# gardnerzhou/CHAP

Measured on AMD Instinct MI355X. Metric: training volumes/sec (2D 256^2 bs24), higher is better.
Workload: dtype bf16; 1 GPU; ACDC 2D DualDecoder bs=24 (12 lab + 12 unlab) 256x256, 1 perturb step(s), N_v=U; global_batch=24, parallelism=dp1, hip_graph=True, losses_finite=True

## Files before the change

### chap_amd/_lib.py

```python
import ctypes as C
import os

_HERE = os.path.dirname(os.path.abspath(__file__))
LIB_PATH = os.environ.get("CHAP_LIBPATH") or os.path.join(_HERE, "libchap_hip.so")

F32, BF16 = 0, 1
STATS_MAX_SLOTS, STATS_HDR = 1024, 4
ACT_BWD_SLOTS = 1024
LOSS_SLOTS, CHANSUM_SLOTS, L2NORM_SLOTS = 512, 512, 256
PACK_CONV_FWD, PACK_CONV_DGRAD, PACK_DECONV_FWD, PACK_DECONV_DGRAD, PACK_DOWN_DGRAD = range(5)

_vp, _i32, _i64, _f32, _sz = C.c_void_p, C.c_int32, C.c_int64, C.c_float, C.c_size_t


class Src(C.Structure):
    _fields_ = [("ptr", _vp), ("scale", _vp), ("shift", _vp), ("keep", _vp), ("chan_mul", _vp),
                ("C", _i32), ("ld", _i32), ("coff", _i32), ("act", _i32), ("slope", _f32), ("keep_scale", _f32)]


class ConvParams(C.Structure):
    _fields_ = [("src", Src * 2), ("nsrc", _i32), ("combine", _i32),
                ("N", _i32), ("D", _i32), ("H", _i32), ("W", _i32), ("ID", _i32), ("IH", _i32), ("IW", _i32),
                ("ksize", _i32), ("stride", _i32), ("dims", _i32),
                ("wpacked", _vp), ("bias", _vp), ("out", _vp),
# ... 70 lines not shown

class ChanSumParams(C.Structure):
    _fields_ = [("r", Src), ("out", _vp), ("npix", _i64), ("pix_per_sample", _i64), ("dtype", _i32), ("ws", _vp)]


class ClToPlanarParams(C.Structure):
    _fields_ = [("r", Src), ("out", _vp), ("N", _i32), ("P", _i32), ("dtype", _i32)]


class MixLossParams(C.Structure):
    _fields_ = [("logits", _vp), ("target_a", _vp), ("target_b", _vp), ("mask", _vp), ("w_a", _f32), ("w_b", _f32),
                ("acc", _vp), ("loss", _vp), ("dlogits", _vp), ("gscale", _f32), ("accumulate", _i32),
                ("N", _i32), ("C", _i32), ("P", _i32), ("smooth", _f32), ("k_dice", _f32), ("k_ce", _f32), ("gscale_dev", _vp)]


class PseudoParams(C.Structure):
    _fields_ = [("logits1", _vp), ("logits2", _vp), ("soft1", _vp), ("soft2", _vp), ("arg1", _vp), ("arg2", _vp),
                ("knowledge", _vp), ("N", _i32), ("C", _i32), ("P", _i32)]


class KlParams(C.Structure):
    _fields_ = [("logits", _vp * 2), ("target", _vp * 2), ("loss", _vp), ("dlogits", _vp * 2),
                ("gscale", _f32), ("gscale_dev", _vp), ("N", _i32), ("C", _i32), ("P", _i32), ("mode", _i32), ("ws", _vp)]


class EnsembleParams(C.Structure):
    _fields_ = [("logits1", _vp), ("logits2", _vp), ("prob", _vp), ("label", _vp), ("N", _i32), ("C", _i32), ("P", C.c_int64), ("mode", _i32)]


class WindowAccParams(C.Structure):
# ... 34 lines not shown
                ("probs_out", _vp), ("inv_npix", _f32), ("nchunk", _i32), ("B", _i32), ("U", _i32), ("C", _i32),
                ("mode", _i32), ("comp", _i32), ("branch", _i32), ("prob_kind", _i32)]


class FoldParams(C.Structure):
    _fields_ = [("g", _vp), ("mul", _vp), ("out", _vp), ("B", _i32), ("U", _i32), ("C", _i32), ("ld", _i32), ("coff", _i32),
                ("pix_per_sample", _i64), ("dtype", _i32)]


class BoxMixParams(C.Structure):
    _fields_ = [("a", _vp), ("b", _vp), ("out", _vp), ("box", _vp), ("N", _i32), ("H", _i32), ("W", _i32), ("is_i64", _i32), ("D", _i32)]


class BoxMaskParams(C.Structure):
    _fields_ = [("mask", _vp), ("box", _vp), ("N", _i32), ("H", _i32), ("W", _i32), ("D", _i32)]


class LccParams(C.Structure):
    _fields_ = [("labels", _vp), ("out", _vp), ("ws", _vp), ("N", _i32), ("H", _i32), ("W", _i32), ("num_classes", _i32), ("D", _i32)]


class DiffMaskParams(C.Structure):
    _fields_ = [("p1", _vp), ("p2", _vp), ("knowledge", _vp), ("out", _vp), ("pooled_ws", _vp),
                ("N", _i32), ("H", _i32), ("W", _i32), ("scale", _i32), ("k", _i32)]


class MetricResult(C.Structure):
    _fields_ = [("n_a", _i64), ("n_b", _i64), ("n_ab", _i64), ("n_ab_s", _i64), ("n_ba_s", _i64), ("q_lo", _i64), ("q_hi", _i64),
                ("sum_ab", C.c_double), ("sum_ba", C.c_double), ("max2_ab", C.c_double), ("max2_ba", C.c_double),
                ("v2_lo", C.c_double), ("v2_hi", C.c_double)]
# ... 41 lines not shown
_SIGS = {
    "chap_conv_fwd": ConvParams, "chap_pack_weights": PackParams, "chap_conv_c1_fwd": ConvC1Params,
    "chap_conv_c1_bwd": ConvC1BwdParams, "chap_wgrad": WgradParams, "chap_bn_finalize": BnFinalizeParams,
    "chap_bn_eval_affine": BnEvalParams, "chap_act_bwd_reduce": ActBwdParams, "chap_act_bwd_apply": ActBwdParams,
    "chap_act_pool2": PoolParams, "chap_upsample2x": UpsampleParams, "chap_upsample2x_bwd": UpsampleBwdParams,
    "chap_planar_to_cl": PlanarToClParams, "chap_channel_sum": ChanSumParams, "chap_cl_to_planar": ClToPlanarParams,
    "chap_ensemble_argmax": EnsembleParams, "chap_window_accumulate": WindowAccParams, "chap_window_finalize": WindowFinParams,
    "chap_mix_loss_fwd": MixLossParams, "chap_mix_loss_bwd": MixLossParams, "chap_pseudo_block": PseudoParams,
    "chap_kl_fwd_bwd": KlParams, "chap_l2_normalize": L2NormParams, "chap_perturb": AxpyParams,
    "chap_rand_uniform": RandParams, "chap_keep_mask": KeepMaskParams, "chap_chan_mask": ChanMaskParams,
    "chap_box_mix": BoxMixParams, "chap_box_mask": BoxMaskParams, "chap_largest_cc": LccParams,
    "chap_diff_mask": DiffMaskParams, "chap_sgd_step": SgdParams,
    "chap_sample_channel_sum": SampleChanSumParams, "chap_channel_drop": ChannelDropParams,
    "chap_fold_perturbed": FoldParams, "chap_grad_sim": GradSimParams, "chap_metrics": MetricsParams,
    "chap_augment2d": Augment2dParams, "chap_augment3d": Augment3dParams,
}
_SIZE_FNS = {"chap_pack_size": PackParams, "chap_conv_c1_bwd_ws": ConvC1BwdParams, "chap_wgrad_ws": WgradParams,
             "chap_lcc_ws": LccParams, "chap_metrics_ws": MetricsParams}

_lib = None


ABI_VERSION = 9


class ChapError(RuntimeError):
    pass


def lib():
# ... 134 lines not shown
```

### chap_amd/csrc/aux.hip

```cpp
#include "common.h"
#include "launch.h"

__global__ __launch_bounds__(256) void l2norm_sumsq_kernel(const float* __restrict__ in, float* __restrict__ ss, int P) {
    __shared__ float red[4];
    const float* x = in + (long)blockIdx.y * P;
    float s = 0.f;
    for (int i = blockIdx.x * 256 + threadIdx.x; i < P; i += gridDim.x * 256) { const float v = x[i]; s += v * v; }
    s = wave_sum(s);
    if ((threadIdx.x & 63) == 0) red[threadIdx.x >> 6] = s;
    __syncthreads();
    if (threadIdx.x == 0) ss[(long)blockIdx.y * CHAP_L2NORM_SLOTS + blockIdx.x] = (red[0] + red[1]) + (red[2] + red[3]);
}
__global__ __launch_bounds__(256) void l2norm_scale_kernel(const float* __restrict__ in, float* __restrict__ out, const float* __restrict__ ss, int P, float eps) {
    __shared__ float tot;
    if (threadIdx.x < 64) {
        double t = 0.0;
        for (int b = threadIdx.x; b < (int)gridDim.x; b += 64) t += (double)ss[(long)blockIdx.y * CHAP_L2NORM_SLOTS + b];
#pragma unroll
        for (int o = 32; o > 0; o >>= 1) t += __shfl_xor(t, o, 64);
        if (threadIdx.x == 0) tot = (float)t;
    }
    __syncthreads();
    const float inv = 1.f / (sqrtf(tot) + eps);
    const float* x = in + (long)blockIdx.y * P;
// ... 101 lines not shown
__global__ void boxmask_kernel(const chap_boxmask_params P, int D) {
    const long total = (long)P.N * D * P.H * P.W;
    for (long i = (long)blockIdx.x * blockDim.x + threadIdx.x; i < total; i += (long)gridDim.x * blockDim.x) {
        const unsigned ui = (unsigned)i;
        const int x = (int)(ui % (unsigned)P.W), y = (int)((ui / (unsigned)P.W) % (unsigned)P.H), z = (int)((ui / (unsigned)(P.W * P.H)) % (unsigned)D);
        P.mask[i] = in_box(P.box, D, z, y, x) ? 0 : 1;
    }
}
extern "C" int chap_box_mask(const chap_boxmask_params* p, void* stream) {
    CHAP_CHECK_ARG(p && p->mask && p->box, "chap_box_mask: null argument");
    const int D = p->D > 1 ? p->D : 1;
    const long total = (long)p->N * D * p->H * p->W;
    const int nb = chap_blocks(total, 2048);
    hipLaunchKernelGGL(boxmask_kernel, dim3(nb), dim3(256), 0, (hipStream_t)stream, *p, D);
    CHAP_LAUNCH_CHECK("chap_box_mask");
    return CHAP_OK;
}

__global__ void diffmask_pool_kernel(const chap_diffmask_params P) {
    const int PH = P.H / P.scale, PW = P.W / P.scale;
    const long total = (long)P.N * PH * PW;
    for (long i = (long)blockIdx.x * blockDim.x + threadIdx.x; i < total; i += (long)gridDim.x * blockDim.x) {
        const int px = (int)(i % PW), py = (int)((i / PW) % PH), n = (int)(i / ((long)PW * PH));
        float s = 0.f;
        for (int dy = 0; dy < P.scale; ++dy)
            for (int dx = 0; dx < P.scale; ++dx) s += P.knowledge[((long)n * P.H + py * P.scale + dy) * P.W + px * P.scale + dx];
        P.pooled_ws[i] = s / (float)(P.scale * P.scale);
    }
}
__global__ __launch_bounds__(1024) void diffmask_select_kernel(const chap_diffmask_params P, float* thr_out) {
// ... 149 lines not shown
```

### chap_amd/csrc/loss.hip

```cpp
#include "common.h"

__device__ __forceinline__ double wave_sum_f64(double v) {
#pragma unroll
    for (int o = 32; o > 0; o >>= 1) v += __shfl_xor(v, o, 64);
    return v;
}
__device__ __forceinline__ void sum_partial_rows(float* ws, int nrows, int rl, float* tot) {
    const int wave = threadIdx.x >> 6, lane = threadIdx.x & 63;
    if (rl <= 32 && nrows <= CHAP_LOSS_SLOTS) {
        constexpr int NR = 8, NB = CHAP_LOSS_SLOTS / 64;
        float v[NR][NB];
#pragma unroll
        for (int r = 0; r < NR; ++r) {
            const int i = wave + 4 * r;
#pragma unroll
            for (int k = 0; k < NB; ++k) {
                const int b = lane + 64 * k;
                v[r][k] = ws[(long)(1 + (b < nrows ? b : 0)) * rl + (i < rl ? i : 0)];
            }
        }
#pragma unroll
        for (int r = 0; r < NR; ++r) {
            const int i = wave + 4 * r;
            double t = 0.0;
// ... 18 lines not shown
template <int C>
__device__ __forceinline__ void softmax_px(const float* __restrict__ lg, long base, long P, float z[C], float p[C], float& lse) {
    float m = -INFINITY;
#pragma unroll
    for (int c = 0; c < C; ++c) { z[c] = lg[base + c * P]; m = fmaxf(m, z[c]); }
    float s = 0.f;
#pragma unroll
    for (int c = 0; c < C; ++c) { p[c] = expf(z[c] - m); s += p[c]; }
    const float inv = 1.f / s;
#pragma unroll
    for (int c = 0; c < C; ++c) p[c] *= inv;
    lse = m + logf(s);
}

template <int C>
__global__ __launch_bounds__(256) void mix_loss_acc_kernel(const chap_mix_loss_params P_) {
    constexpr int NA = 2 + 3 * C;
    __shared__ float red[4][2 * NA];
    float a[2][NA];
#pragma unroll
    for (int k = 0; k < 2; ++k)
#pragma unroll
        for (int i = 0; i < NA; ++i) a[k][i] = 0.f;
    const long P = P_.P, total = (long)P_.N * P;
    for (long i = (long)blockIdx.x * 256 + threadIdx.x; i < total; i += (long)gridDim.x * 256) {
        const long n = (unsigned)i / (unsigned)P, pp = (unsigned)i % (unsigned)P;
        float z[C], p[C], lse;
        softmax_px<C>(P_.logits, n * C * P + pp, P, z, p, lse);
        const float m = P_.mask ? (float)P_.mask[i] : 1.f;
        const int t[2] = {(int)P_.target_a[i], (int)(P_.target_b ? P_.target_b[i] : P_.target_a[i])};
        const float mk[2] = {m, 1.f - m};
#pragma unroll
        for (int k = 0; k < 2; ++k) {
            float zt = 0.f;
#pragma unroll
            for (int c = 0; c < C; ++c) {
                const float tc = (t[k] == c) ? 1.f : 0.f;
                zt += tc * z[c];
                a[k][1 + c] += p[c] * tc * mk[k];
                a[k][1 + C + c] += p[c] * p[c] * mk[k];
                a[k][1 + 2 * C + c] += tc * mk[k];
            }
            a[k][0] += (lse - zt) * mk[k];
            a[k][1 + 3 * C] += mk[k];
        }
    }
#pragma unroll
    for (int k = 0; k < 2; ++k)
#pragma unroll
        for (int i = 0; i < NA; ++i) {
            const float v = wave_sum(a[k][i]);
            if ((threadIdx.x & 63) == 0) red[threadIdx.x >> 6][k * NA + i] = v;
        }
    __syncthreads();
    for (int i = threadIdx.x; i < 2 * NA; i += 256) P_.acc[(long)(1 + blockIdx.x) * 2 * NA + i] = (red[0][i] + red[1][i]) + (red[2][i] + red[3][i]);
}

__global__ __launch_bounds__(256) void mix_loss_final_kernel(float* acc, int nblocks, float* loss, int C, float w_a, float w_b, float smooth, float k_dice, float k_ce) {
    __shared__ float tot[2 * (2 + 3 * 8)];
    const int NA = 2 + 3 * C;
    sum_partial_rows(acc, nblocks, 2 * NA, tot);
    if (threadIdx.x != 0) return;
    float part[2];
    const float w[2] = {w_a, w_b};
    for (int k = 0; k < 2; ++k) {
        const float* a = tot + k * NA;
        float dice = 0.f;
        for (int c = 0; c < C; ++c) dice += 1.f - (2.f * a[1 + c] + smooth) / (a[1 + C + c] + a[1 + 2 * C + c] + smooth);
        dice = dice / C * w[k];
        const float ce = w[k] * a[0] / (a[1 + 3 * C] + 1e-16f);
        part[k] = k_dice * dice + k_ce * ce;
    }
    loss[0] = part[0]; loss[1] = part[1]; loss[2] = part[0] + part[1];
}

template <int C>
__global__ __launch_bounds__(256) void mix_loss_bwd_kernel(const chap_mix_loss_params P_) {
    constexpr int NA = 2 + 3 * C;
    __shared__ float sa[2 * NA];
    for (int i = threadIdx.x; i < 2 * NA; i += 256) sa[i] = P_.acc[i];
    __syncthreads();
    const long P = P_.P, total = (long)P_.N * P;
    const float w[2] = {P_.w_a, P_.w_b};
    const float gsc = P_.gscale * (P_.gscale_dev ? *P_.gscale_dev : 1.f);
    for (long i = (long)blockIdx.x * 256 + threadIdx.x; i < total; i += (long)gridDim.x * 256) {
        const long n = (unsigned)i / (unsigned)P, pp = (unsigned)i % (unsigned)P;
        float z[C], p[C], lse;
        softmax_px<C>(P_.logits, n * C * P + pp, P, z, p, lse);
        const float m = P_.mask ? (float)P_.mask[i] : 1.f;
        const int t[2] = {(int)P_.target_a[i], (int)(P_.target_b ? P_.target_b[i] : P_.target_a[i])};
        const float mk[2] = {m, 1.f - m};
        const bool dflt = P_.k_dice == 0.f && P_.k_ce == 0.f;
        const float kd = dflt ? 0.5f : P_.k_dice, kc = dflt ? 0.5f : P_.k_ce;
        float dz[C], dp[C];
#pragma unroll
        for (int c = 0; c < C; ++c) { dz[c] = 0.f; dp[c] = 0.f; }
#pragma unroll
        for (int k = 0; k < 2; ++k) {
            const float* a = sa + k * NA;
            const float kce = w[k] * mk[k] / (a[1 + 3 * C] + 1e-16f);
// ... 4 lines not shown
                const float den = a[1 + C + c] + a[1 + 2 * C + c] + P_.smooth;
                dp[c] += (w[k] / C) * mk[k] * (-2.f * tc / den + (2.f * a[1 + c] + P_.smooth) * 2.f * p[c] / (den * den));
            }
        }
        float dot = 0.f;
#pragma unroll
        for (int c = 0; c < C; ++c) dot += dp[c] * p[c];
#pragma unroll
        for (int c = 0; c < C; ++c) {
            const float gz = gsc * (kc * dz[c] + kd * p[c] * (dp[c] - dot));
            float* o = P_.dlogits + n * C * P + c * P + pp;
            *o = P_.accumulate ? *o + gz : gz;
        }
    }
}

static int loss_blocks(long total) { long b = (total + 255) / 256; return (int)(b < 2048 ? b : 2048); }
static int loss_slots(long total) { long b = (total + 255) / 256; return (int)(b < CHAP_LOSS_SLOTS ? b : CHAP_LOSS_SLOTS); }

extern "C" int chap_mix_loss_fwd(const chap_mix_loss_params* p, void* stream) {
    CHAP_CHECK_ARG(p && p->logits && p->target_a && p->acc && p->loss, "chap_mix_loss_fwd: null argument");
    CHAP_CHECK_ARG(p->C == 4 || p->C == 2, "chap_mix_loss: C=%d (2 or 4 built)", p->C);
    CHAP_CHECK_ARG((long)p->N * p->P < (1L << 32), "chap_mix_loss: N*P=%ld exceeds the 32-bit pixel index", (long)p->N * p->P);
    const int nb = loss_slots((long)p->N * p->P);
    hipStream_t s = (hipStream_t)stream;
    if (p->C == 4) hipLaunchKernelGGL(mix_loss_acc_kernel<4>, dim3(nb), dim3(256), 0, s, *p);
    else hipLaunchKernelGGL(mix_loss_acc_kernel<2>, dim3(nb), dim3(256), 0, s, *p);
    CHAP_LAUNCH_CHECK("chap_mix_loss_fwd");
    const bool dflt = p->k_dice == 0.f && p->k_ce == 0.f;
    hipLaunchKernelGGL(mix_loss_final_kernel, dim3(1), dim3(256), 0, s, p->acc, nb, p->loss, p->C, p->w_a, p->w_b, p->smooth,
                       dflt ? 0.5f : p->k_dice, dflt ? 0.5f : p->k_ce);
    CHAP_LAUNCH_CHECK("chap_mix_loss_fwd(final)");
    return CHAP_OK;
}
extern "C" int chap_mix_loss_bwd(const chap_mix_loss_params* p, void* stream) {
    CHAP_CHECK_ARG(p && p->logits && p->target_a && p->acc && p->dlogits, "chap_mix_loss_bwd: null argument");
    CHAP_CHECK_ARG(p->C == 4 || p->C == 2, "chap_mix_loss: C=%d (2 or 4 built)", p->C);
    CHAP_CHECK_ARG((long)p->N * p->P < (1L << 32), "chap_mix_loss: N*P=%ld exceeds the 32-bit pixel index", (long)p->N * p->P);
    const int nb = loss_blocks((long)p->N * p->P);
    if (p->C == 4) hipLaunchKernelGGL(mix_loss_bwd_kernel<4>, dim3(nb), dim3(256), 0, (hipStream_t)stream, *p);
    else hipLaunchKernelGGL(mix_loss_bwd_kernel<2>, dim3(nb), dim3(256), 0, (hipStream_t)stream, *p);
    CHAP_LAUNCH_CHECK("chap_mix_loss_bwd");
    return CHAP_OK;
}

template <int C>
__global__ __launch_bounds__(256) void pseudo_kernel(const chap_pseudo_params P_) {
    const long P = P_.P, total = (long)P_.N * P;
    for (long i = (long)blockIdx.x * 256 + threadIdx.x; i < total; i += (long)gridDim.x * 256) {
        const long n = (unsigned)i / (unsigned)P, pp = (unsigned)i % (unsigned)P, base = n * C * P + pp;
        float z1[C], p1[C], l1, z2[C], p2[C], l2;
        softmax_px<C>(P_.logits1, base, P, z1, p1, l1);
        softmax_px<C>(P_.logits2, base, P, z2, p2, l2);
        int a1 = 0, a2 = 0;
#pragma unroll
        for (int c = 1; c < C; ++c) { if (p1[c] > p1[a1]) a1 = c; if (p2[c] > p2[a2]) a2 = c; }
        if (P_.soft1) {
// ... 293 lines not shown
```

### chap_amd/csrc/metrics.hip

```cpp
#include <climits>
#include <cmath>
#include "common.h"

namespace {

constexpr int MET_TB = 256;
constexpr int MET_LDS_BUDGET = 40960;
constexpr int MET_RC_MAX = 8;

__device__ __forceinline__ int64_t met_ld(const void* p, int is64, unsigned i) {
    return is64 ? ((const int64_t*)p)[i] : (int64_t)((const uint8_t*)p)[i];
}

__device__ __forceinline__ int met_border(const void* X, int is64, int binary, const int64_t* cls, int K, unsigned i,
                                          int d, int h, int w, int D, int H, int W, int ndim, bool& border) {
    const int64_t v = met_ld(X, is64, i);
    int k = -1;
    if (binary) k = v != 0 ? 0 : -1;
    else for (int c = 0; c < K; ++c) if (cls[c] == v) { k = c; break; }
    border = false;
    if (k < 0) return k;
    const unsigned HW = (unsigned)H * (unsigned)W;
#define MET_OUT(cond, j) (cond) || (binary ? met_ld(X, is64, (j)) == 0 : met_ld(X, is64, (j)) != v)
    border = MET_OUT(w == 0, i - 1) || MET_OUT(w == W - 1, i + 1) || MET_OUT(h == 0, i - W) || MET_OUT(h == H - 1, i + W);
// ... 302 lines not shown
int met_cols(hipStream_t s, double* dist, int F, int n, long stride, int W, int O1, long ostride, long V, double sp) {
    if (n <= 1) return CHAP_OK;
    int TW = 16;
    while (TW > 1 && (long)n * TW * (long)sizeof(double) > MET_LDS_BUDGET) TW >>= 1;
    const int T = MET_TB / TW, per = (n + T - 1) / T;
    const int rounds = (per + MET_RC_MAX - 1) / MET_RC_MAX, rc = (per + rounds - 1) / rounds;
    const int ntw = (W + TW - 1) / TW;
    const dim3 grid((unsigned)((long)F * O1 * ntw));
    const size_t lds = (size_t)n * TW * sizeof(double);
    switch (rc) {
#define MET_RC(R) case R: met_launch_cols<R>(grid, lds, s, dist, n, stride, W, O1, ostride, V, TW, ntw, sp); break;
        MET_RC(1) MET_RC(2) MET_RC(3) MET_RC(4) MET_RC(5) MET_RC(6) MET_RC(7) MET_RC(8)
#undef MET_RC
        default: chap_set_error("chap_metrics: internal error (rc %d)", rc); return CHAP_EINVAL;
    }
    CHAP_LAUNCH_CHECK("chap_metrics(edt)");
    return CHAP_OK;
}

int met_check(const chap_metrics_params* p) {
    CHAP_CHECK_ARG(p && p->a && p->b && p->border_a && p->border_b && p->results, "chap_metrics: null argument");
    CHAP_CHECK_ARG(p->K >= 1 && p->K <= 255, "chap_metrics: K must be in [1, 255] (got %d)", p ? p->K : 0);
    CHAP_CHECK_ARG(p->binary ? p->K == 1 : p->classes != nullptr, "chap_metrics: binary needs K == 1, class mode a class list");
    CHAP_CHECK_ARG(p->ndim == 3 || (p->ndim == 2 && p->D == 1), "chap_metrics: ndim must be 3, or 2 with D == 1");
    CHAP_CHECK_ARG(p->D >= 1 && p->H >= 1 && p->W >= 1, "chap_metrics: empty shape");
    CHAP_CHECK_ARG(p->D <= CHAP_METRICS_MAX_AXIS && p->H <= CHAP_METRICS_MAX_AXIS && p->W <= CHAP_METRICS_MAX_AXIS,
                   "chap_metrics: axis longer than CHAP_METRICS_MAX_AXIS (%d): D=%d H=%d W=%d", CHAP_METRICS_MAX_AXIS, p->D, p->H, p->W);
    CHAP_CHECK_ARG((long)p->D * p->H * p->W < (1L << 31), "chap_metrics: more than 2^31 - 1 voxels");
    CHAP_CHECK_ARG(p->a_i64 == 0 || p->a_i64 == 1, "chap_metrics: a_i64 must be 0 or 1");
    CHAP_CHECK_ARG(p->b_i64 == 0 || p->b_i64 == 1, "chap_metrics: b_i64 must be 0 or 1");
// ... 56 lines not shown
```

### chap_amd/ops.py

```python
import torch

from . import _lib as L


def _stream():
    return torch.cuda.current_stream().cuda_stream


def dt(t):
    if t.dtype == torch.float32:
        return L.F32
    if t.dtype == torch.bfloat16:
        return L.BF16
    raise TypeError("unsupported activation dtype %s" % t.dtype)


def _p(t):
    return None if t is None else t.data_ptr()


class Lazy:

    __slots__ = ("raw", "C", "coff", "scale", "shift", "act", "slope", "keep", "keep_scale", "chan_mul")

# ... 234 lines not shown
    L.call("chap_mix_loss_fwd", p, _stream())
    return loss, acc


def mix_loss_bwd(logits, target_a, target_b, mask, w_a, w_b, acc, dlogits, gscale=1.0, accumulate=False, smooth=1e-10, k_dice=0.0, k_ce=0.0,
                 gscale_dev=None):
    N, Cc = logits.shape[0], logits.shape[1]
    p = L.MixLossParams()
    p.logits, p.target_a, p.target_b, p.mask = logits.data_ptr(), target_a.data_ptr(), _p(target_b), _p(mask)
    p.w_a, p.w_b, p.acc, p.dlogits = w_a, w_b, acc.data_ptr(), dlogits.data_ptr()
    p.gscale, p.accumulate, p.gscale_dev = gscale, int(accumulate), _p(gscale_dev)
    p.N, p.C, p.P, p.smooth, p.k_dice, p.k_ce = N, Cc, logits[0, 0].numel(), smooth, k_dice, k_ce
    L.call("chap_mix_loss_bwd", p, _stream())


def pseudo_block(logits1, logits2, want_soft=True):
    N, Cc = logits1.shape[0], logits1.shape[1]
    sp = logits1.shape[2:]
    dev = logits1.device
    soft1 = L.hold_empty_like(logits1) if want_soft else None
    soft2 = L.hold_empty_like(logits2) if want_soft else None
    arg1 = L.hold_empty((N,) + tuple(sp), dtype=torch.int64, device=dev)
    arg2 = L.hold_empty_like(arg1)
    know = L.hold_empty((N,) + tuple(sp), dtype=torch.float32, device=dev)
    p = L.PseudoParams()
    p.logits1, p.logits2, p.soft1, p.soft2 = logits1.data_ptr(), logits2.data_ptr(), _p(soft1), _p(soft2)
    p.arg1, p.arg2, p.knowledge = arg1.data_ptr(), arg2.data_ptr(), know.data_ptr()
    p.N, p.C, p.P = N, Cc, logits1[0, 0].numel()
    L.call("chap_pseudo_block", p, _stream())
    return soft1, soft2, arg1, arg2, know


DIST_MODES = {"kl": 0, "dice": 1}


def kl_fwd_bwd(logits, targets, loss, dlogits=(None, None), gscale=1.0, gscale_dev=None, mode="kl"):
    p = L.KlParams()
    p.mode = DIST_MODES[mode]
# ... 70 lines not shown
    p = L.FoldParams()
    out = L.hold_empty((B,) + tuple(g.shape[1:-1]) + (Cc,), dtype=g.dtype, device=g.device)
    p.g, p.mul, p.out = g.data_ptr(), _p(mul), out.data_ptr()
    p.B, p.U, p.C, p.ld, p.coff = B, U, Cc, g.shape[-1], coff
    p.pix_per_sample, p.dtype = g[0, ..., 0].numel(), dt(g)
    L.call("chap_fold_perturbed", p, _stream())
    return out


def box_mix(a, b, out, box):
    p = L.BoxMixParams()
    p.a, p.b, p.out, p.box = a.data_ptr(), b.data_ptr(), out.data_ptr(), box.data_ptr()
    p.N, p.H, p.W, p.is_i64 = a.shape[0], a.shape[-2], a.shape[-1], int(a.dtype == torch.int64)
    p.D = a.shape[-3] if box.numel() == 6 else 1
    L.call("chap_box_mix", p, _stream())


def box_mask(mask, box):
    p = L.BoxMaskParams()
    p.mask, p.box, p.N, p.H, p.W = mask.data_ptr(), box.data_ptr(), mask.shape[0], mask.shape[-2], mask.shape[-1]
    p.D = mask.shape[-3] if box.numel() == 6 else 1
    L.call("chap_box_mask", p, _stream())


def largest_cc(labels, num_classes):
    out = L.hold_empty_like(labels)
    p = L.LccParams()
    p.labels, p.out = labels.data_ptr(), out.data_ptr()
    p.N, p.H, p.W, p.num_classes = labels.shape[0], labels.shape[-2], labels.shape[-1], num_classes
    p.D = labels.shape[1] if labels.dim() == 4 else 1
# ... 113 lines not shown
```

### chap_amd/train.py

```python
import contextlib
import math
import os

import numpy as np
import torch

from . import ops


def sigmoid_rampup(current, rampup_length):
    if rampup_length == 0:
        return 1.0
    t = float(np.clip(current, 0.0, rampup_length)) / rampup_length
    return float(math.exp(-5.0 * (1.0 - t) ** 2))


def get_current_consistency_weight(epoch, args):
    return args["consistency"] * sigmoid_rampup(epoch, args["consistency_rampup"])


DEFAULT_ARGS = dict(base_lr=0.01, batch_size=24, labeled_bs=12, max_iterations=30000, num_classes=4,
                    consistency=1.0, consistency_rampup=50.0, noise_mag=10.0, epi=6.0, topk1=0.1,
                    adv_noise=True, adv_losstype="kl", vat_iters=1, vat_sign=False, nms=1,
                    momentum=0.9, weight_decay=1e-4, dropout=False, comp_drop=False)
# ... 174 lines not shown
        self.world_size = world_size
        self.grad_sync = None
        self._graph, self._graph_opt, self._graphs_dp = None, None, None
        self.sim_score = None
        self.gradsim = None
        if a["dropout"] and self.dims == 2:
            self.gradsim = GradSim(dev, a["num_classes"])
            self.gradsim.init_simsocre(model)
            n_ = model.flat_buffers()[1].numel()
            self._grad_lu = torch.zeros(2 * n_, dtype=torch.float32, device=dev)
        n = model.flat_buffers()[1].numel()
        self.grad_both = torch.zeros(2 * n, dtype=torch.float32, device=dev)
        model.swap_grad_buffer(self.grad_both[:n])
        self.grad2 = self.grad_both[n:]
        self.concurrent = bool(a.get("concurrent", True))
        st = _distinct_streams(dev, 4)
        self._cap = st[3]
        self._side = st[0] if self.concurrent else None
        self._d2 = st[1] if self.concurrent else None
        self._pre = st[2] if self.concurrent else None

    def prepare(self, box_yx=None):
        a = self.args
        sizes = [int(s * 2 / 3) for s in self._hw]
        if box_yx is None:
            box_yx = tuple(np.random.randint(0, s - p) for s, p in zip(self._hw, sizes))
        self._upload_sched(list(box_yx) + sizes, get_current_consistency_weight(self.iter_num // 150, a))

    def _upload_sched(self, box_vals, cw):
        import struct
# ... 133 lines not shown
                next(gen)
            except StopIteration as e:
                return e.value

    def _phase_b(self, ctx):
        return self._drain(self._phase_b_steps(ctx))

    def _phase_v(self, ctx):
        return self._drain(self._phase_v_steps(ctx))

    def _phase_b_steps(self, ctx):
        a, model, inject = self.args, self.model, ctx["inject"]
        nc = a["num_classes"]
        lsub, usub, volume_batch = ctx["lsub"], ctx["usub"], ctx["volume_batch"]
        with torch.no_grad():
            if a["nms"]:
                plab1 = ops.largest_cc(ctx["pseudo_outputs1"], nc)
                plab2 = ops.largest_cc(ctx["pseudo_outputs2"], nc)
            else:
                plab1, plab2 = ctx["pseudo_outputs1"], ctx["pseudo_outputs2"]
            loss_mask = torch.empty(lsub, *volume_batch.shape[2:], dtype=torch.int64, device=volume_batch.device)
            ops.box_mask(loss_mask, self.box)
            net_input_mix = torch.empty((lsub + usub,) + tuple(volume_batch.shape[1:]), dtype=torch.float32, device=volume_batch.device)
            ops.box_mix(ctx["img_b"], ctx["uimg_b"], net_input_mix[:lsub], self.box)
            ops.box_mix(ctx["uimg_a"], ctx["img_a"], net_input_mix[lsub:], self.box)
        lab_a, lab_b = ctx["lab_a"], ctx["lab_b"]
        plab_a1, plab_b1 = plab1[:usub], plab1[usub:]
        plab_a2, plab_b2 = plab2[:usub], plab2[usub:]
        out_mix1, out_mix2 = model(net_input_mix, drop_masks=inject.get("drop_B"))
        d1, d2 = torch.empty_like(out_mix1), torch.empty_like(out_mix2)
        terms = (
            (out_mix1[lsub:], d1[lsub:], plab_a2, lab_a, True),
            (out_mix2[lsub:], d2[lsub:], plab_a1, lab_a, True),
            (out_mix1[:lsub], d1[:lsub], lab_b, plab_b2, False),
            (out_mix2[:lsub], d2[:lsub], lab_b, plab_b1, False),
        )
        losses = []
        split = self.gradsim is not None and inject.get("sim_score") is None and self.sim_score is None
        if split:
            e1, e2 = torch.empty_like(out_mix1), torch.empty_like(out_mix2)
            eterms = (e1[lsub:], e2[lsub:], e1[:lsub], e2[:lsub])
        for ti, (lg, dl, img_l, patch_l, unlab) in enumerate(terms):
            iw, pw = (0.5, 1.0) if unlab else (1.0, 0.5)
            loss3, acc = ops.mix_loss_fwd(lg, img_l, patch_l, loss_mask, iw, pw)
            if split:
                wl, wu = ((0.0, pw), (iw, 0.0)) if unlab else ((iw, 0.0), (0.0, pw))
                ops.mix_loss_bwd(lg, img_l, patch_l, loss_mask, wl[0], wl[1], acc, dl)
                ops.mix_loss_bwd(lg, img_l, patch_l, loss_mask, wu[0], wu[1], acc, eterms[ti])
            else:
                ops.mix_loss_bwd(lg, img_l, patch_l, loss_mask, iw, pw, acc, dl)
            losses.append(loss3)
        yield
        if not split:
            torch.autograd.backward([out_mix1, out_mix2], [d1, d2])
            return losses
        n_ = self._grad_lu.numel() // 2
        g_l, g_u = self._grad_lu[:n_], self._grad_lu[n_:]
# ... 217 lines not shown
```

### include/chap_hip.h

```cpp
#ifndef CHAP_HIP_H
#define CHAP_HIP_H

#include <stddef.h>
#include <stdint.h>

#ifdef __cplusplus
extern "C" {
#endif

#define CHAP_ABI_VERSION 9
#define CHAP_STATS_MAX_SLOTS 1024
#define CHAP_STATS_HDR 4
#define CHAP_ACT_BWD_SLOTS 1024
#define CHAP_LOSS_SLOTS 512
#define CHAP_CHANSUM_SLOTS 512
#define CHAP_L2NORM_SLOTS 256

enum { CHAP_F32 = 0, CHAP_BF16 = 1 };
enum { CHAP_OK = 0, CHAP_EINVAL = -1, CHAP_EUNSUPPORTED = -2, CHAP_ELAUNCH = -3 };

typedef struct {
    const void*    ptr;
    const float*   scale;
    const float*   shift;
// ... 160 lines not shown
    const float* logits;
    const int64_t* target_a;
    const int64_t* target_b;
    const int64_t* mask;
    float w_a, w_b;
    float* acc;
    float* loss;
    float* dlogits;
    float gscale; int32_t accumulate;
    int32_t N, C, P; float smooth;
    float k_dice, k_ce;
    const float* gscale_dev;
} chap_mix_loss_params;
int chap_mix_loss_fwd(const chap_mix_loss_params* p, void* stream);
int chap_mix_loss_bwd(const chap_mix_loss_params* p, void* stream);

typedef struct {
    const float* logits1; const float* logits2;
    float* soft1; float* soft2;
    int64_t* arg1; int64_t* arg2;
    float* knowledge;
    int32_t N, C, P;
} chap_pseudo_params;
int chap_pseudo_block(const chap_pseudo_params* p, void* stream);

typedef struct {
    const float* logits[2]; const float* target[2];
    float* loss;  float* dlogits[2];
    float gscale; const float* gscale_dev;
    int32_t N, C, P;
// ... 5 lines not shown
typedef struct { const float* in; float* out; int32_t N, P; float eps; float* ws;  } chap_l2norm_params;
int chap_l2_normalize(const chap_l2norm_params* p, void* stream);
typedef struct { const float* x; const float* d; const float* mask; float* out; float alpha; int32_t sign; int64_t n; } chap_axpy_params;
int chap_perturb(const chap_axpy_params* p, void* stream);
typedef struct { float* out; uint64_t seed; const uint64_t* seed_dev; int64_t n; float lo, hi; } chap_rand_params;
int chap_rand_uniform(const chap_rand_params* p, void* stream);
typedef struct { uint8_t* keep; uint64_t seed; const uint64_t* seed_dev; int64_t n; float p; } chap_keepmask_params;
int chap_keep_mask(const chap_keepmask_params* p, void* stream);
typedef struct { float* mul; uint64_t seed; const uint64_t* seed_dev; int64_t n; float p; } chap_chanmask_params;
int chap_chan_mask(const chap_chanmask_params* p, void* stream);

typedef struct { const void* a; const void* b; void* out; const int32_t* box; int32_t N, H, W; int32_t is_i64; int32_t D; } chap_boxmix_params;
int chap_box_mix(const chap_boxmix_params* p, void* stream);
typedef struct { int64_t* mask; const int32_t* box; int32_t N, H, W, D; } chap_boxmask_params;
int chap_box_mask(const chap_boxmask_params* p, void* stream);

typedef struct { const int64_t* labels; int64_t* out; void* ws; int32_t N, H, W, num_classes; int32_t D;  } chap_lcc_params;
size_t chap_lcc_ws(const chap_lcc_params* p);
int    chap_largest_cc(const chap_lcc_params* p, void* stream);

typedef struct { const int64_t* p1; const int64_t* p2; const float* knowledge; float* out; float* pooled_ws;
                 int32_t N, H, W, scale; int32_t k; } chap_diffmask_params;
int chap_diff_mask(const chap_diffmask_params* p, void* stream);

typedef struct { float* param; float* grad; float* grad2 ; float* mom; const float* lr;
                 float momentum, weight_decay, grad_scale; int64_t n; int32_t zero_grad; } chap_sgd_params;
int chap_sgd_step(const chap_sgd_params* p, void* stream);

typedef struct { const float* logits1; const float* logits2; float* prob ; uint8_t* label ;
                 int32_t N, C; int64_t P; int32_t mode; } chap_ensemble_params;
// ... 101 lines not shown
```

Measured before the change: 3989 volumes/s.

## Batch pass-B loss terms, box mixes and largest-CC into fewer launches

Adds multi-term mix-loss forward/backward kernels that process up to four loss terms in one grid (blockIdx.y selects the term). Also adds a fused kernel that writes the box mask and both box-mixed inputs in one pass. Pseudo-label argmax outputs now share one buffer so largest-CC can run once on the stacked pair. The aim is to cut kernel launch count and small-kernel tail overhead in the BCP pass. The cost is that blocks beyond a term's slot count exit early, and the new path is gated by a passb_batch flag that defaults to the concurrent setting.

```diff
diff --git a/chap_amd/_lib.py b/chap_amd/_lib.py
--- a/chap_amd/_lib.py
+++ b/chap_amd/_lib.py
@@ -108,6 +108,10 @@
                 ("N", _i32), ("C", _i32), ("P", _i32), ("smooth", _f32), ("k_dice", _f32), ("k_ce", _f32), ("gscale_dev", _vp)]
 
 
+class MixLossMultiParams(C.Structure):
+    _fields_ = [("nterms", _i32), ("term", MixLossParams * 4)]
+
+
 class PseudoParams(C.Structure):
     _fields_ = [("logits1", _vp), ("logits2", _vp), ("soft1", _vp), ("soft2", _vp), ("arg1", _vp), ("arg2", _vp),
                 ("knowledge", _vp), ("N", _i32), ("C", _i32), ("P", _i32)]
@@ -172,6 +176,10 @@
 
 class BoxMaskParams(C.Structure):
     _fields_ = [("mask", _vp), ("box", _vp), ("N", _i32), ("H", _i32), ("W", _i32), ("D", _i32)]
+
+
+class BcpMixParams(C.Structure):
+    _fields_ = [("a", _vp * 2), ("b", _vp * 2), ("out", _vp * 2), ("mask", _vp), ("box", _vp), ("N", _i32 * 2), ("Nm", _i32), ("H", _i32), ("W", _i32), ("D", _i32)]
 
 
 class LccParams(C.Structure):
@@ -243,6 +251,7 @@
     "chap_sample_channel_sum": SampleChanSumParams, "chap_channel_drop": ChannelDropParams,
     "chap_fold_perturbed": FoldParams, "chap_grad_sim": GradSimParams, "chap_metrics": MetricsParams,
     "chap_augment2d": Augment2dParams, "chap_augment3d": Augment3dParams,
+    "chap_mix_loss_multi_fwd": MixLossMultiParams, "chap_mix_loss_multi_bwd": MixLossMultiParams, "chap_bcp_mix": BcpMixParams,
 }
 _SIZE_FNS = {"chap_pack_size": PackParams, "chap_conv_c1_bwd_ws": ConvC1BwdParams, "chap_wgrad_ws": WgradParams,
              "chap_lcc_ws": LccParams, "chap_metrics_ws": MetricsParams}
diff --git a/chap_amd/csrc/aux.hip b/chap_amd/csrc/aux.hip
--- a/chap_amd/csrc/aux.hip
+++ b/chap_amd/csrc/aux.hip
@@ -139,6 +139,31 @@
     const int nb = chap_blocks(total, 2048);
     hipLaunchKernelGGL(boxmask_kernel, dim3(nb), dim3(256), 0, (hipStream_t)stream, *p, D);
     CHAP_LAUNCH_CHECK("chap_box_mask");
+    return CHAP_OK;
+}
+__global__ void bcpmix_kernel(const chap_bcpmix_params P, int D) {
+    const long vol = (long)D * P.H * P.W, n0 = P.N[0] * vol, n1 = n0 + P.N[1] * vol, total = n1 + P.Nm * vol;
+    for (long i = (long)blockIdx.x * blockDim.x + threadIdx.x; i < total; i += (long)gridDim.x * blockDim.x) {
+        const int part = i < n0 ? 0 : i < n1 ? 1 : 2;
+        const long j = i - (part == 0 ? 0 : part == 1 ? n0 : n1);
+        const unsigned uj = (unsigned)j;
+        const int x = (int)(uj % (unsigned)P.W), y = (int)((uj / (unsigned)P.W) % (unsigned)P.H), z = (int)((uj / (unsigned)(P.W * P.H)) % (unsigned)D);
+        const bool in = in_box(P.box, D, z, y, x);
+        if (part == 2) P.mask[j] = in ? 0 : 1;
+        else (part ? P.out[1] : P.out[0])[j] = in ? (part ? P.b[1] : P.b[0])[j] : (part ? P.a[1] : P.a[0])[j];
+    }
+}
+extern "C" int chap_bcp_mix(const chap_bcpmix_params* p, void* stream) {
+    CHAP_CHECK_ARG(p && p->a[0] && p->b[0] && p->out[0] && p->a[1] && p->b[1] && p->out[1] && p->mask && p->box, "chap_bcp_mix: null argument");
+    CHAP_CHECK_ARG(p->N[0] > 0 && p->N[1] > 0 && p->Nm > 0 && p->H > 0 && p->W > 0, "chap_bcp_mix: empty argument");
+    const int D = p->D > 1 ? p->D : 1;
+    const long vol = (long)D * p->H * p->W;
+    const long most = (long)(p->N[0] > p->N[1] ? (p->N[0] > p->Nm ? p->N[0] : p->Nm) : (p->N[1] > p->Nm ? p->N[1] : p->Nm)) * vol;
+    CHAP_CHECK_ARG(most < (1L << 32), "chap_bcp_mix: %ld elements in one part exceed the 32-bit element index", most);
+    const long total = ((long)p->N[0] + p->N[1] + p->Nm) * vol;
+    const int nb = chap_blocks(total, 2048);
+    hipLaunchKernelGGL(bcpmix_kernel, dim3(nb), dim3(256), 0, (hipStream_t)stream, *p, D);
+    CHAP_LAUNCH_CHECK("chap_bcp_mix");
     return CHAP_OK;
 }
 
diff --git a/chap_amd/csrc/loss.hip b/chap_amd/csrc/loss.hip
--- a/chap_amd/csrc/loss.hip
+++ b/chap_amd/csrc/loss.hip
@@ -56,7 +56,7 @@
 }
 
 template <int C>
-__global__ __launch_bounds__(256) void mix_loss_acc_kernel(const chap_mix_loss_params P_) {
+__device__ __forceinline__ void mix_loss_acc_body(const chap_mix_loss_params& P_, const int blk, const int nblk) {
     constexpr int NA = 2 + 3 * C;
     __shared__ float red[4][2 * NA];
     float a[2][NA];
@@ -65,7 +65,7 @@
 #pragma unroll
         for (int i = 0; i < NA; ++i) a[k][i] = 0.f;
     const long P = P_.P, total = (long)P_.N * P;
-    for (long i = (long)blockIdx.x * 256 + threadIdx.x; i < total; i += (long)gridDim.x * 256) {
+    for (long i = (long)blk * 256 + threadIdx.x; i < total; i += (long)nblk * 256) {
         const long n = (unsigned)i / (unsigned)P, pp = (unsigned)i % (unsigned)P;
         float z[C], p[C], lse;
         softmax_px<C>(P_.logits, n * C * P + pp, P, z, p, lse);
@@ -95,10 +95,12 @@
             if ((threadIdx.x & 63) == 0) red[threadIdx.x >> 6][k * NA + i] = v;
         }
     __syncthreads();
-    for (int i = threadIdx.x; i < 2 * NA; i += 256) P_.acc[(long)(1 + blockIdx.x) * 2 * NA + i] = (red[0][i] + red[1][i]) + (red[2][i] + red[3][i]);
-}
-
-__global__ __launch_bounds__(256) void mix_loss_final_kernel(float* acc, int nblocks, float* loss, int C, float w_a, float w_b, float smooth, float k_dice, float k_ce) {
+    for (int i = threadIdx.x; i < 2 * NA; i += 256) P_.acc[(long)(1 + blk) * 2 * NA + i] = (red[0][i] + red[1][i]) + (red[2][i] + red[3][i]);
+}
+template <int C>
+__global__ __launch_bounds__(256) void mix_loss_acc_kernel(const chap_mix_loss_params P_) { mix_loss_acc_body<C>(P_, blockIdx.x, gridDim.x); }
+
+__device__ __forceinline__ void mix_loss_final_body(float* acc, int nblocks, float* loss, int C, float w_a, float w_b, float smooth, float k_dice, float k_ce) {
     __shared__ float tot[2 * (2 + 3 * 8)];
     const int NA = 2 + 3 * C;
     sum_partial_rows(acc, nblocks, 2 * NA, tot);
@@ -115,9 +117,12 @@
     }
     loss[0] = part[0]; loss[1] = part[1]; loss[2] = part[0] + part[1];
 }
-
-template <int C>
-__global__ __launch_bounds__(256) void mix_loss_bwd_kernel(const chap_mix_loss_params P_) {
+__global__ __launch_bounds__(256) void mix_loss_final_kernel(float* acc, int nblocks, float* loss, int C, float w_a, float w_b, float smooth, float k_dice, float k_ce) {
+    mix_loss_final_body(acc, nblocks, loss, C, w_a, w_b, smooth, k_dice, k_ce);
+}
+
+template <int C>
+__device__ __forceinline__ void mix_loss_bwd_body(const chap_mix_loss_params& P_, const int blk, const int nblk) {
     constexpr int NA = 2 + 3 * C;
     __shared__ float sa[2 * NA];
     for (int i = threadIdx.x; i < 2 * NA; i += 256) sa[i] = P_.acc[i];
@@ -125,7 +130,7 @@
     const long P = P_.P, total = (long)P_.N * P;
     const float w[2] = {P_.w_a, P_.w_b};
     const float gsc = P_.gscale * (P_.gscale_dev ? *P_.gscale_dev : 1.f);
-    for (long i = (long)blockIdx.x * 256 + threadIdx.x; i < total; i += (long)gridDim.x * 256) {
+    for (long i = (long)blk * 256 + threadIdx.x; i < total; i += (long)nblk * 256) {
         const long n = (unsigned)i / (unsigned)P, pp = (unsigned)i % (unsigned)P;
         float z[C], p[C], lse;
         softmax_px<C>(P_.logits, n * C * P + pp, P, z, p, lse);
@@ -160,9 +165,32 @@
         }
     }
 }
-
-static int loss_blocks(long total) { long b = (total + 255) / 256; return (int)(b < 2048 ? b : 2048); }
-static int loss_slots(long total) { long b = (total + 255) / 256; return (int)(b < CHAP_LOSS_SLOTS ? b : CHAP_LOSS_SLOTS); }
+template <int C>
+__global__ __launch_bounds__(256) void mix_loss_bwd_kernel(const chap_mix_loss_params P_) { mix_loss_bwd_body<C>(P_, blockIdx.x, gridDim.x); }
+
+constexpr int LOSS_MAX_BLOCKS = 2048;
+__host__ __device__ inline int loss_blocks(long total) { long b = (total + 255) / 256; return (int)(b < LOSS_MAX_BLOCKS ? b : LOSS_MAX_BLOCKS); }
+__host__ __device__ inline int loss_slots(long total) { long b = (total + 255) / 256; return (int)(b < CHAP_LOSS_SLOTS ? b : CHAP_LOSS_SLOTS); }
+
+template <int C>
+__global__ __launch_bounds__(256) void mix_loss_multi_acc_kernel(const chap_mix_loss_multi_params M) {
+    const chap_mix_loss_params& P_ = M.term[blockIdx.y];
+    const int nb = loss_slots((long)P_.N * P_.P);
+    if ((int)blockIdx.x >= nb) return;
+    mix_loss_acc_body<C>(P_, blockIdx.x, nb);
+}
+__global__ __launch_bounds__(256) void mix_loss_multi_final_kernel(const chap_mix_loss_multi_params M) {
+    const chap_mix_loss_params& P_ = M.term[blockIdx.x];
+    const bool dflt = P_.k_dice == 0.f && P_.k_ce == 0.f;
+    mix_loss_final_body(P_.acc, loss_slots((long)P_.N * P_.P), P_.loss, P_.C, P_.w_a, P_.w_b, P_.smooth, dflt ? 0.5f : P_.k_dice, dflt ? 0.5f : P_.k_ce);
+}
+template <int C>
+__global__ __launch_bounds__(256) void mix_loss_multi_bwd_kernel(const chap_mix_loss_multi_params M) {
+    const chap_mix_loss_params& P_ = M.term[blockIdx.y];
+    const int nb = loss_blocks((long)P_.N * P_.P);
+    if ((int)blockIdx.x >= nb) return;
+    mix_loss_bwd_body<C>(P_, blockIdx.x, nb);
+}
 
 extern "C" int chap_mix_loss_fwd(const chap_mix_loss_params* p, void* stream) {
     CHAP_CHECK_ARG(p && p->logits && p->target_a && p->acc && p->loss, "chap_mix_loss_fwd: null argument");
@@ -187,6 +215,42 @@
     if (p->C == 4) hipLaunchKernelGGL(mix_loss_bwd_kernel<4>, dim3(nb), dim3(256), 0, (hipStream_t)stream, *p);
     else hipLaunchKernelGGL(mix_loss_bwd_kernel<2>, dim3(nb), dim3(256), 0, (hipStream_t)stream, *p);
     CHAP_LAUNCH_CHECK("chap_mix_loss_bwd");
+    return CHAP_OK;
+}
+
+static int mix_loss_multi_check(const chap_mix_loss_multi_params* m, bool bwd, const char* who) {
+    CHAP_CHECK_ARG(m, "%s: null argument", who);
+    CHAP_CHECK_ARG(m->nterms >= 1 && m->nterms <= 4, "%s: nterms=%d (1..4)", who, m->nterms);
+    for (int t = 0; t < m->nterms; ++t) {
+        const chap_mix_loss_params* p = &m->term[t];
+        CHAP_CHECK_ARG(p->logits && p->target_a && p->acc && (bwd ? (const void*)p->dlogits : (const void*)p->loss), "%s: null argument in term %d", who, t);
+        CHAP_CHECK_ARG(p->C == 4 || p->C == 2, "chap_mix_loss: C=%d (2 or 4 built)", p->C);
+        CHAP_CHECK_ARG(p->C == m->term[0].C && p->P == m->term[0].P, "%s: term %d has C=%d P=%d, term 0 C=%d P=%d (C and P are common)", who, t, p->C, p->P,
+                       m->term[0].C, m->term[0].P);
+        CHAP_CHECK_ARG(p->N > 0 && p->P > 0, "%s: term %d is empty (N=%d P=%d)", who, t, p->N, p->P);
+        CHAP_CHECK_ARG((long)p->N * p->P < (1L << 32), "chap_mix_loss: N*P=%ld exceeds the 32-bit pixel index", (long)p->N * p->P);
+    }
+    return CHAP_OK;
+}
+extern "C" int chap_mix_loss_multi_fwd(const chap_mix_loss_multi_params* m, void* stream) {
+    if (const int rc = mix_loss_multi_check(m, false, "chap_mix_loss_multi_fwd")) return rc;
+    int nb = 0;
+    for (int t = 0; t < m->nterms; ++t) { const int n = loss_slots((long)m->term[t].N * m->term[t].P); nb = n > nb ? n : nb; }
+    hipStream_t s = (hipStream_t)stream;
+    if (m->term[0].C == 4) hipLaunchKernelGGL(mix_loss_multi_acc_kernel<4>, dim3(nb, m->nterms), dim3(256), 0, s, *m);
+    else hipLaunchKernelGGL(mix_loss_multi_acc_kernel<2>, dim3(nb, m->nterms), dim3(256), 0, s, *m);
+    CHAP_LAUNCH_CHECK("chap_mix_loss_multi_fwd");
+    hipLaunchKernelGGL(mix_loss_multi_final_kernel, dim3(m->nterms), dim3(256), 0, s, *m);
+    CHAP_LAUNCH_CHECK("chap_mix_loss_multi_fwd(final)");
+    return CHAP_OK;
+}
+extern "C" int chap_mix_loss_multi_bwd(const chap_mix_loss_multi_params* m, void* stream) {
+    if (const int rc = mix_loss_multi_check(m, true, "chap_mix_loss_multi_bwd")) return rc;
+    int nb = 0;
+    for (int t = 0; t < m->nterms; ++t) { const int n = loss_blocks((long)m->term[t].N * m->term[t].P); nb = n > nb ? n : nb; }
+    if (m->term[0].C == 4) hipLaunchKernelGGL(mix_loss_multi_bwd_kernel<4>, dim3(nb, m->nterms), dim3(256), 0, (hipStream_t)stream, *m);
+    else hipLaunchKernelGGL(mix_loss_multi_bwd_kernel<2>, dim3(nb, m->nterms), dim3(256), 0, (hipStream_t)stream, *m);
+    CHAP_LAUNCH_CHECK("chap_mix_loss_multi_bwd");
     return CHAP_OK;
 }
 
diff --git a/chap_amd/csrc/metrics.hip b/chap_amd/csrc/metrics.hip
--- a/chap_amd/csrc/metrics.hip
+++ b/chap_amd/csrc/metrics.hip
@@ -340,6 +340,8 @@
 #undef MET_RC
         default: chap_set_error("chap_metrics: internal error (rc %d)", rc); return CHAP_EINVAL;
     }
+    void* const stream = (void*)s;
+    (void)stream;
     CHAP_LAUNCH_CHECK("chap_metrics(edt)");
     return CHAP_OK;
 }
diff --git a/chap_amd/ops.py b/chap_amd/ops.py
--- a/chap_amd/ops.py
+++ b/chap_amd/ops.py
@@ -272,14 +272,49 @@
     L.call("chap_mix_loss_bwd", p, _stream())
 
 
+def _fill_mix_loss(p, logits, target_a, target_b, mask, w_a, w_b, acc, smooth, k_dice, k_ce):
+    p.logits, p.target_a, p.target_b, p.mask = logits.data_ptr(), target_a.data_ptr(), _p(target_b), _p(mask)
+    p.w_a, p.w_b, p.acc = w_a, w_b, acc.data_ptr()
+    p.N, p.C, p.P, p.smooth, p.k_dice, p.k_ce = logits.shape[0], logits.shape[1], logits[0, 0].numel(), smooth, k_dice, k_ce
+
+
+def mix_loss_multi_fwd(terms):
+    m = L.MixLossMultiParams()
+    m.nterms = len(terms)
+    if not 1 <= len(terms) <= 4:
+        raise ValueError("mix_loss_multi_fwd: %d terms (1..4)" % len(terms))
+    res = []
+    for p, t in zip(m.term, terms):
+        lg = t["logits"]
+        acc = L.hold_empty((1 + L.LOSS_SLOTS) * 2 * (2 + 3 * lg.shape[1]), dtype=torch.float32, device=lg.device)
+        loss = L.hold_empty(3, dtype=torch.float32, device=lg.device)
+        _fill_mix_loss(p, lg, t["target_a"], t.get("target_b"), t.get("mask"), t["w_a"], t["w_b"], acc, t.get("smooth", 1e-10), t.get("k_dice", 0.0), t.get("k_ce", 0.0))
+        p.loss = loss.data_ptr()
+        res.append((loss, acc))
+    L.call("chap_mix_loss_multi_fwd", m, _stream())
+    return res
+
+
+def mix_loss_multi_bwd(terms):
+    m = L.MixLossMultiParams()
+    m.nterms = len(terms)
+    if not 1 <= len(terms) <= 4:
+        raise ValueError("mix_loss_multi_bwd: %d terms (1..4)" % len(terms))
+    for p, t in zip(m.term, terms):
+        _fill_mix_loss(p, t["logits"], t["target_a"], t.get("target_b"), t.get("mask"), t["w_a"], t["w_b"], t["acc"], t.get("smooth", 1e-10),
+                       t.get("k_dice", 0.0), t.get("k_ce", 0.0))
+        p.dlogits, p.gscale, p.accumulate, p.gscale_dev = t["dlogits"].data_ptr(), t.get("gscale", 1.0), int(t.get("accumulate", False)), _p(t.get("gscale_dev"))
+    L.call("chap_mix_loss_multi_bwd", m, _stream())
+
+
 def pseudo_block(logits1, logits2, want_soft=True):
     N, Cc = logits1.shape[0], logits1.shape[1]
     sp = logits1.shape[2:]
     dev = logits1.device
     soft1 = L.hold_empty_like(logits1) if want_soft else None
     soft2 = L.hold_empty_like(logits2) if want_soft else None
-    arg1 = L.hold_empty((N,) + tuple(sp), dtype=torch.int64, device=dev)
-    arg2 = L.hold_empty_like(arg1)
+    arg = L.hold_empty((2 * N,) + tuple(sp), dtype=torch.int64, device=dev)
+    arg1, arg2 = arg[:N], arg[N:]
     know = L.hold_empty((N,) + tuple(sp), dtype=torch.float32, device=dev)
     p = L.PseudoParams()
     p.logits1, p.logits2, p.soft1, p.soft2 = logits1.data_ptr(), logits2.data_ptr(), _p(soft1), _p(soft2)
@@ -380,6 +415,24 @@
     p.N, p.H, p.W, p.is_i64 = a.shape[0], a.shape[-2], a.shape[-1], int(a.dtype == torch.int64)
     p.D = a.shape[-3] if box.numel() == 6 else 1
     L.call("chap_box_mix", p, _stream())
+
+
+def bcp_mix(a0, b0, out0, a1, b1, out1, mask, box):
+    p = L.BcpMixParams()
+    for h, (a, b, o) in enumerate(((a0, b0, out0), (a1, b1, out1))):
+        assert a.dtype == b.dtype == o.dtype == torch.float32 and a.shape == b.shape == o.shape and a.shape[-2:] == mask.shape[-2:]
+        p.a[h], p.b[h], p.out[h], p.N[h] = a.data_ptr(), b.data_ptr(), o.data_ptr(), a.shape[0]
+    p.mask, p.box, p.Nm, p.H, p.W = mask.data_ptr(), box.data_ptr(), mask.shape[0], mask.shape[-2], mask.shape[-1]
+    p.D = mask.shape[-3] if box.numel() == 6 else 1
+    L.call("chap_bcp_mix", p, _stream())
+
+
+def _stacked_pair(a, b):
+    base = a._base
+    if base is None or b._base is not base or not base.is_contiguous() or base.shape[0] != 2 * a.shape[0] or base.shape[1:] != a.shape[1:]:
+        return None
+    n = a.numel() * a.element_size()
+    return base if (a.shape == b.shape and a.data_ptr() == base.data_ptr() and b.data_ptr() == base.data_ptr() + n) else None
 
 
 def box_mask(mask, box):
diff --git a/chap_amd/train.py b/chap_amd/train.py
--- a/chap_amd/train.py
+++ b/chap_amd/train.py
@@ -212,6 +212,8 @@
         model.swap_grad_buffer(self.grad_both[:n])
         self.grad2 = self.grad_both[n:]
         self.concurrent = bool(a.get("concurrent", True))
+        pb = a.get("passb_batch")
+        self.passb_batch = self.concurrent if pb is None else bool(pb)
         st = _distinct_streams(dev, 4)
         self._cap = st[3]
         self._side = st[0] if self.concurrent else None
@@ -375,16 +377,24 @@
         nc = a["num_classes"]
         lsub, usub, volume_batch = ctx["lsub"], ctx["usub"], ctx["volume_batch"]
         with torch.no_grad():
-            if a["nms"]:
+            batch = self.passb_batch
+            stacked = ops._stacked_pair(ctx["pseudo_outputs1"], ctx["pseudo_outputs2"]) if (batch and a["nms"]) else None
+            if stacked is not None:
+                plab = ops.largest_cc(stacked, nc)
+                plab1, plab2 = plab[:plab.shape[0] // 2], plab[plab.shape[0] // 2:]
+            elif a["nms"]:
                 plab1 = ops.largest_cc(ctx["pseudo_outputs1"], nc)
                 plab2 = ops.largest_cc(ctx["pseudo_outputs2"], nc)
             else:
                 plab1, plab2 = ctx["pseudo_outputs1"], ctx["pseudo_outputs2"]
             loss_mask = torch.empty(lsub, *volume_batch.shape[2:], dtype=torch.int64, device=volume_batch.device)
-            ops.box_mask(loss_mask, self.box)
             net_input_mix = torch.empty((lsub + usub,) + tuple(volume_batch.shape[1:]), dtype=torch.float32, device=volume_batch.device)
-            ops.box_mix(ctx["img_b"], ctx["uimg_b"], net_input_mix[:lsub], self.box)
-            ops.box_mix(ctx["uimg_a"], ctx["img_a"], net_input_mix[lsub:], self.box)
+            if batch:
+                ops.bcp_mix(ctx["img_b"], ctx["uimg_b"], net_input_mix[:lsub], ctx["uimg_a"], ctx["img_a"], net_input_mix[lsub:], loss_mask, self.box)
+            else:
+                ops.box_mask(loss_mask, self.box)
+                ops.box_mix(ctx["img_b"], ctx["uimg_b"], net_input_mix[:lsub], self.box)
+                ops.box_mix(ctx["uimg_a"], ctx["img_a"], net_input_mix[lsub:], self.box)
         lab_a, lab_b = ctx["lab_a"], ctx["lab_b"]
         plab_a1, plab_b1 = plab1[:usub], plab1[usub:]
         plab_a2, plab_b2 = plab2[:usub], plab2[usub:]
@@ -401,7 +411,20 @@
         if split:
             e1, e2 = torch.empty_like(out_mix1), torch.empty_like(out_mix2)
             eterms = (e1[lsub:], e2[lsub:], e1[:lsub], e2[:lsub])
-        for ti, (lg, dl, img_l, patch_l, unlab) in enumerate(terms):
+        if batch:
+            base = [dict(logits=lg, target_a=img_l, target_b=patch_l, mask=loss_mask) for lg, _, img_l, patch_l, _ in terms]
+            wts = [(0.5, 1.0) if unlab else (1.0, 0.5) for *_, unlab in terms]
+            fwd = ops.mix_loss_multi_fwd([dict(b, w_a=iw, w_b=pw) for b, (iw, pw) in zip(base, wts)])
+            losses = [l for l, _ in fwd]
+            bwd = lambda ws, outs: ops.mix_loss_multi_bwd([dict(b, w_a=w[0], w_b=w[1], acc=acc, dlogits=o) for b, w, (_, acc), o in zip(base, ws, fwd, outs)])
+            if split:
+                wl = [(0.0, pw) if unlab else (iw, 0.0) for (iw, pw), (*_, unlab) in zip(wts, terms)]
+                wu = [(iw, 0.0) if unlab else (0.0, pw) for (iw, pw), (*_, unlab) in zip(wts, terms)]
+                bwd(wl, [t[1] for t in terms])
+                bwd(wu, eterms)
+            else:
+                bwd(wts, [t[1] for t in terms])
+        for ti, (lg, dl, img_l, patch_l, unlab) in enumerate(() if batch else terms):
             iw, pw = (0.5, 1.0) if unlab else (1.0, 0.5)
             loss3, acc = ops.mix_loss_fwd(lg, img_l, patch_l, loss_mask, iw, pw)
             if split:
diff --git a/include/chap_hip.h b/include/chap_hip.h
--- a/include/chap_hip.h
+++ b/include/chap_hip.h
@@ -198,6 +198,9 @@
 } chap_mix_loss_params;
 int chap_mix_loss_fwd(const chap_mix_loss_params* p, void* stream);
 int chap_mix_loss_bwd(const chap_mix_loss_params* p, void* stream);
+typedef struct { int32_t nterms; chap_mix_loss_params term[4]; } chap_mix_loss_multi_params;
+int chap_mix_loss_multi_fwd(const chap_mix_loss_multi_params* p, void* stream);
+int chap_mix_loss_multi_bwd(const chap_mix_loss_multi_params* p, void* stream);
 
 typedef struct {
     const float* logits1; const float* logits2;
@@ -233,6 +236,8 @@
 int chap_box_mix(const chap_boxmix_params* p, void* stream);
 typedef struct { int64_t* mask; const int32_t* box; int32_t N, H, W, D; } chap_boxmask_params;
 int chap_box_mask(const chap_boxmask_params* p, void* stream);
+typedef struct { const float* a[2]; const float* b[2]; float* out[2]; int64_t* mask; const int32_t* box; int32_t N[2]; int32_t Nm, H, W, D; } chap_bcpmix_params;
+int chap_bcp_mix(const chap_bcpmix_params* p, void* stream);
 
 typedef struct { const int64_t* labels; int64_t* out; void* ws; int32_t N, H, W, num_classes; int32_t D;  } chap_lcc_params;
 size_t chap_lcc_ws(const chap_lcc_params* p);
```

Measured after the change: 4041 volumes/s (median of 6 runs). 1.01x the previous value.
